# snt-arg/visual_sgraphs

Hardware: NVIDIA B200
Metric: orb_extraction_frames_per_s_640x480_1000f (higher is better)
Workload: dtype u8

## Files before the change

visual_sgraphs_b200/csrc/fast.cu:

```cuda
#include "blur_device.cuh"
#include "vsg_internal.cuh"

namespace vsg {

__device__ __forceinline__ uint32_t min2(uint32_t a, uint32_t b) { uint32_t d; asm("min.u16x2 %0, %1, %2;" : "=r"(d) : "r"(a), "r"(b)); return d; }
__device__ __forceinline__ uint32_t max2(uint32_t a, uint32_t b) { uint32_t d; asm("max.u16x2 %0, %1, %2;" : "=r"(d) : "r"(a), "r"(b)); return d; }
__device__ __forceinline__ uint32_t min3(uint32_t a, uint32_t b, uint32_t c) { return min2(min2(a, b), c); }
__device__ __forceinline__ uint32_t max3(uint32_t a, uint32_t b, uint32_t c) { return max2(max2(a, b), c); }

constexpr int kFastThreads = 160;
#ifndef VSG_FAST_MINB
#define VSG_FAST_MINB 6
#endif
constexpr int kT2Pitch = 52;
constexpr int kS2Pitch = 52;
constexpr int kMaxS = 28;

__device__ __forceinline__ uint32_t fast_strength2(const uint32_t *c) {
    constexpr int P = kT2Pitch;
    uint32_t p[16];
    p[0] = c[3 * P];       p[1] = c[3 * P + 1];    p[2] = c[2 * P + 2];    p[3] = c[P + 3];
    p[4] = c[3];           p[5] = c[-P + 3];       p[6] = c[-2 * P + 2];   p[7] = c[-3 * P + 1];
    p[8] = c[-3 * P];      p[9] = c[-3 * P - 1];   p[10] = c[-2 * P - 2];  p[11] = c[-P - 3];
    p[12] = c[-3];         p[13] = c[P - 3];       p[14] = c[2 * P - 2];   p[15] = c[3 * P - 1];
    const uint32_t v = c[0];
    uint32_t glo[4], ghi[4];
#pragma unroll
    for (int g = 0; g < 4; ++g) {
        const int b = 4 * g;
        const uint32_t s0 = p[b], s1 = p[b + 1], s2 = p[b + 2], s3 = p[(b + 9) & 15], s4 = p[(b + 10) & 15], s5 = p[(b + 11) & 15];
        const uint32_t q0 = p[b + 3], q1 = p[(b + 4) & 15], q2 = p[(b + 5) & 15], q3 = p[(b + 6) & 15], q4 = p[(b + 7) & 15], q5 = p[(b + 8) & 15];
        glo[g] = min3(max2(min3(max2(s0, s3), s1, s2), min3(max2(s2, s5), s3, s4)), min3(q0, q1, q2), min3(q3, q4, q5));
        ghi[g] = max3(min2(max3(min2(s0, s3), s1, s2), max3(min2(s2, s5), s3, s4)), max3(q0, q1, q2), max3(q3, q4, q5));
    }
    const uint32_t best_lo = max3(glo[0], glo[1], max2(glo[2], glo[3]));
    const uint32_t best_hi = min3(ghi[0], ghi[1], min2(ghi[2], ghi[3]));
    return max2(max2(best_lo, v) - v, v - min2(best_hi, v));
}

__constant__ uint32_t kRcpS[kMaxS / 4 + 1] = {0u, 0x40000000u, 0x20000000u, 0x15555556u, 0x10000000u, 0x0CCCCCCDu, 0x0AAAAAABu, 0x0924924Au};
__constant__ uint8_t kRowsPerSweep[kMaxS / 4 + 1] = {0, 40, 20, 13, 10, 8, 6, 5};

struct CellGeom {
    int level, x0, y0, cw, ch;
};
__device__ __forceinline__ CellGeom cell_geom(const FrameGeom &g, int cell_block) {
    CellGeom c;
    int level = 0;
#pragma unroll
    for (int l = 1; l < 8; ++l) level += cell_block >= g.lv[l].cell_begin ? 1 : 0;
    for (int l = 8; l < g.nlevels; ++l) level += cell_block >= g.lv[l].cell_begin ? 1 : 0;
    const LevelGeom &L = g.lv[level];
    const int local = cell_block - L.cell_begin;
    const int ci = (int)__umulhi((uint32_t)local, L.cols_rcp), cj = local - ci * L.cols_eff;
    c.level = level;
    c.x0 = kBorderMin + cj * L.w_cell;
    c.y0 = kBorderMin + ci * L.h_cell;
    c.cw = min(c.x0 + L.w_cell + 6, L.w - kBorderMin) - c.x0;
    c.ch = min(c.y0 + L.h_cell + 6, L.h - kBorderMin) - c.y0;
    return c;
}

__device__ __forceinline__ void fast_cell_body(const FrameGeom &g, const CellGeom &cell, const uint8_t *__restrict__ lvl0_base,
                                               int lvl0_pitch, int64_t lvl0_stride, const uint8_t *__restrict__ pyr,
                                               uint32_t *t2, uint32_t *s2, uint32_t *list, Cand *__restrict__ cand,
                                               int *__restrict__ cand_count, int ini_th, int min_th, int list_cap, int frame) {
    __shared__ int s_count, s_base;
    const int level = cell.level, x0 = cell.x0, y0 = cell.y0, cw = cell.cw, ch = cell.ch;
    const LevelGeom &L = g.lv[level];
    const int tid = threadIdx.x;
    const int iw = cw - 6, ih = ch - 6;
    const int S = (((iw + 1) >> 1) + 3) & ~3;
    const int ax0 = x0 & ~3;
    const int xoff = x0 - ax0;
    {
        const int nq = (xoff + S + 6 + 3) >> 2;
        const int lq = nq <= 8 ? 3 : 4;
        const int q = tid & ((1 << lq) - 1), r0 = tid >> lq, rstep = kFastThreads >> lq;
        const bool qok = q < nq;
        auto relayout = [&](uint32_t a, uint32_t b, uint32_t *dst) {
            uint4 o;
            o.x = __byte_perm(a, b, 0x7470) & 0x00FF00FFu;
            o.y = __byte_perm(a, b, 0x7571) & 0x00FF00FFu;
            o.z = __byte_perm(a, b, 0x7672) & 0x00FF00FFu;
            o.w = __byte_perm(a, b, 0x7773) & 0x00FF00FFu;
            *reinterpret_cast<uint4 *>(dst) = o;
        };
        const uint8_t *src;
        int spitch;
        if (level == 0) { src = lvl0_base + (int64_t)frame * lvl0_stride; spitch = lvl0_pitch; }
        else { src = pyr + L.plane_offset + (int64_t)frame * L.plane_stride; spitch = L.pitch; }
        const uint8_t *base = src + (int64_t)y0 * spitch + ax0;
        const uint8_t *row = base + (int64_t)r0 * spitch + 4 * q;
        const int64_t rinc = (int64_t)rstep * spitch;
        uint32_t *dst = t2 + r0 * kT2Pitch + 4 * q;
        constexpr int kLoadIters = 3;
        uint32_t a[kLoadIters], b[kLoadIters];
#pragma unroll
        for (int it = 0; it < kLoadIters; ++it) {
            if (qok && r0 + it * rstep < ch) {
                a[it] = __ldg(reinterpret_cast<const uint32_t *>(row + it * rinc));
                b[it] = __ldg(reinterpret_cast<const uint32_t *>(row + it * rinc + S));
            }
        }
#pragma unroll
        for (int it = 0; it < kLoadIters; ++it)
            if (qok && r0 + it * rstep < ch) relayout(a[it], b[it], dst + it * rstep * kT2Pitch);
        for (int r = r0 + kLoadIters * rstep; qok && r < ch; r += rstep) {
            const uint8_t *rp = base + (int64_t)r * spitch + 4 * q;
            relayout(__ldg(reinterpret_cast<const uint32_t *>(rp)), __ldg(reinterpret_cast<const uint32_t *>(rp + S)),
                     t2 + r * kT2Pitch + 4 * q);
        }
    }
    for (int i = tid; i < kS2Pitch; i += kFastThreads) {
        s2[i] = 0;
        s2[(ih + 1) * kS2Pitch + i] = 0;
    }
    if (tid == 0) s_count = 0;

    const int RB = kRowsPerSweep[S >> 2];
    const int trow = (int)__umulhi((uint32_t)tid, kRcpS[S >> 2]);
    const int j = tid - trow * S;
    const int row0 = trow < RB ? trow : ih;
    const uint32_t kmask = (j < iw ? 0x0000FFFFu : 0u) | (j + S < iw ? 0xFFFF0000u : 0u);
    __syncthreads();

    {
        const uint32_t *c = t2 + (3 + row0) * kT2Pitch + xoff + 3 + j;
        uint32_t *k = s2 + (row0 + 1) * kS2Pitch + j + 1;
        const bool first = j == 0, last = j == S - 1;
        for (int row = row0; row < ih; row += RB, c += RB * kT2Pitch, k += RB * kS2Pitch) {
            const uint32_t K = fast_strength2(c) & kmask;
            *k = K;
            if (last) k[-S] = K << 16;
            if (first) k[S] = K >> 16;
        }
    }
    __syncthreads();

    for (int pass = 0; pass < 2; ++pass) {
        const int t = pass == 0 ? ini_th : min_th;
        const int tt = max(t, 1);
        const uint32_t tt2 = (uint32_t)tt * 0x00010001u;
        uint32_t acc = 0, pw = 1;
        const uint32_t *c = s2 + (row0 + 1) * kS2Pitch + j + 1;
        for (int row = row0; row < ih; row += RB, c += RB * kS2Pitch, pw <<= 1) {
            const uint32_t K = c[0];
            const uint32_t nb = max3(max3(c[-kS2Pitch - 1], c[-kS2Pitch], c[-kS2Pitch + 1]),
                                     max3(c[-1], c[1], c[kS2Pitch - 1]), max3(c[kS2Pitch], c[kS2Pitch + 1], tt2));
            const uint32_t e = K - min2(K, nb);
            acc += min2(e, 0x00010001u) * pw;
        }
        const int cnt = __popc(acc);
        if (cnt) {
            int pos = atomicAdd(&s_count, cnt);
            uint32_t m0 = acc & 0xFFFFu, m1 = acc >> 16;
            const uint32_t *kcol = s2 + (row0 + 1) * kS2Pitch + j + 1;
            while (m0) {
                const int i = __ffs(m0) - 1;
                m0 &= m0 - 1;
                const uint32_t K = kcol[i * RB * kS2Pitch] & 0xFFFFu;
                list[pos++] = (uint32_t)j | ((uint32_t)(row0 + i * RB) << 8) | ((K - 1) << 16);
            }
            while (m1) {
                const int i = __ffs(m1) - 1;
                m1 &= m1 - 1;
                const uint32_t K = kcol[i * RB * kS2Pitch] >> 16;
                list[pos++] = (uint32_t)(j + S) | ((uint32_t)(row0 + i * RB) << 8) | ((K - 1) << 16);
            }
        }
        __syncthreads();
        if (s_count > 0) break;
    }
    const int n = min(s_count, list_cap);
    if (n == 0) return;
    const int slot_idx = frame * g.nlevels + level;
    if (tid == 0) s_base = atomicAdd(&cand_count[slot_idx], n);
    __syncthreads();
    Cand *out = cand + L.cand_offset + (int64_t)frame * g.cand_total;
    for (int i = tid; i < n; i += kFastThreads) {
        const int dst = s_base + i;
        if (dst >= L.cand_cap) break;
        const uint32_t e = list[i];
        Cand c;
        c.x = (unsigned short)(x0 + 3 + (e & 0xff));
        c.y = (unsigned short)(y0 + 3 + ((e >> 8) & 0xff));
        c.score = (unsigned short)(e >> 16);
        c.pad = 0;
        out[dst] = c;
    }
}

struct FastSmem {
    uint32_t *t2, *s2, *list;
};
__device__ __forceinline__ FastSmem fast_smem(uint8_t *base, int tile_rows) {
    FastSmem m;
    m.t2 = reinterpret_cast<uint32_t *>(base);
    m.s2 = m.t2 + tile_rows * kT2Pitch;
    m.list = m.s2 + (tile_rows - 4) * kS2Pitch;
    return m;
}

__global__ void __launch_bounds__(kFastThreads, VSG_FAST_MINB) fast_kernel(FrameGeom g,
                                                             const uint8_t *__restrict__ lvl0_base, int lvl0_pitch,
                                                             int64_t lvl0_stride, const uint8_t *__restrict__ pyr,
                                                             Cand *__restrict__ cand, int *__restrict__ cand_count,
                                                             int ini_th, int min_th, int tile_rows, int list_cap) {
    extern __shared__ __align__(16) uint8_t smem[];
    pdl_launch_dependents();
    pdl_wait();
    const FastSmem m = fast_smem(smem, tile_rows);
    fast_cell_body(g, cell_geom(g, blockIdx.x), lvl0_base, lvl0_pitch, lvl0_stride, pyr, m.t2, m.s2, m.list, cand,
                   cand_count, ini_th, min_th, list_cap, blockIdx.y);
}

struct UnitRole {
    bool blur;
    int index;
};
__device__ __forceinline__ UnitRole unit_role(int x, int nblur, int ratio, uint32_t group_rcp) {
    const int group = ratio + 1;
    UnitRole r;
    if (x < nblur * group) {
        const int gi = group == 1 ? x : (int)__umulhi((uint32_t)x, group_rcp), pos = x - gi * group;
        r.blur = pos == ratio;
        r.index = r.blur ? gi : gi * ratio + pos;
    } else {
        r.blur = false;
        r.index = nblur * ratio + (x - nblur * group);
    }
    return r;
}

__global__ void __launch_bounds__(kFastThreads, VSG_FAST_MINB) fast_blur_kernel(FrameGeom g, BlurLevels bl,
                                                                  const uint8_t *__restrict__ lvl0_base, int lvl0_pitch,
                                                                  int64_t lvl0_stride, const uint8_t *__restrict__ pyr,
                                                                  uint8_t *__restrict__ blur, Cand *__restrict__ cand,
                                                                  int *__restrict__ cand_count, int ini_th, int min_th,
                                                                  int tile_rows, int list_cap, int nblur, int ratio,
                                                                  uint32_t group_rcp) {
    extern __shared__ __align__(16) uint8_t smem[];
    pdl_launch_dependents();
    pdl_wait();
    const UnitRole role = unit_role(blockIdx.x, nblur, ratio, group_rcp);
    if (role.blur) {
        blur_block_body(g, bl, lvl0_base, lvl0_pitch, lvl0_stride, pyr, blur, role.index, blockIdx.y);
        return;
    }
    const FastSmem m = fast_smem(smem, tile_rows);
    fast_cell_body(g, cell_geom(g, role.index), lvl0_base, lvl0_pitch, lvl0_stride, pyr, m.t2, m.s2, m.list, cand,
                   cand_count, ini_th, min_th, list_cap, blockIdx.y);
}

vsg_status launch_fast(const FrameGeom &g, const uint8_t *lvl0_base, int lvl0_pitch, int64_t lvl0_stride, const uint8_t *pyr,
                       uint8_t *blur, Cand *cand, int *cand_count, int ini_th, int min_th, int max_cw, int max_ch, int nframes,
                       cudaStream_t s) {
    if (g.ncells == 0) {
        if (blur) launch_blur(g, lvl0_base, lvl0_pitch, lvl0_stride, pyr, blur, nframes, s);
        return VSG_OK;
    }
    const int max_S = ((((max_cw - 6) + 1) >> 1) + 3) & ~3;
    if (3 + max_S + 6 + 3 > kT2Pitch || max_S + 2 > kS2Pitch || max_S > kMaxS || (max_ch - 6) > 16 * (kFastThreads / max_S)) {
        set_error("FAST cell larger than the shared-memory tile / the 16-sweep survivor masks");
        return VSG_ERR_INVALID;
    }
    const int tile_rows = max_ch;
    const int list_cap = ((max_cw - 6 + 1) / 2) * ((max_ch - 6 + 1) / 2) + 1;
    const size_t smem = (size_t)tile_rows * kT2Pitch * 4 + (size_t)(tile_rows - 4) * kS2Pitch * 4 + (size_t)list_cap * 4 + 16;
    if (smem > 48 * 1024) {
        cudaFuncSetAttribute(fast_kernel, cudaFuncAttributeMaxDynamicSharedMemorySize, (int)smem);
        cudaFuncSetAttribute(fast_blur_kernel, cudaFuncAttributeMaxDynamicSharedMemorySize, (int)smem);
    }
    if (!blur) {
        launch_kernel(fast_kernel, dim3(g.ncells, nframes), dim3(kFastThreads), smem, s, true, g, lvl0_base, lvl0_pitch,
                      lvl0_stride, pyr, cand, cand_count, ini_th, min_th, tile_rows, list_cap);
    } else {
        const BlurLevels bl = make_blur_levels(g, nframes, kFastThreads);
        const int nblur = bl.block_begin[g.nlevels];
        const int ratio = g.ncells / nblur;
        const uint32_t group_rcp = (uint32_t)((0x100000000ull + (uint64_t)ratio) / (uint64_t)(ratio + 1));
        launch_kernel(fast_blur_kernel, dim3(g.ncells + nblur, nframes), dim3(kFastThreads), smem, s, true, g, bl, lvl0_base,
                      lvl0_pitch, lvl0_stride, pyr, blur, cand, cand_count, ini_th, min_th, tile_rows, list_cap, nblur, ratio,
                      group_rcp);
    }
    count_launch();
    return VSG_OK;
}

}
```

visual_sgraphs_b200/csrc/vsg_api.cu:

```cuda
#include <algorithm>
#include <atomic>
#include <cmath>
#include <cstdarg>
#include <cstdio>
#include <cstdlib>
#include <cstring>
#include <vector>

#include "vsg_internal.cuh"

namespace vsg {

static thread_local char g_err[512] = "";
static std::atomic<int64_t> g_launches{0};

void set_error(const char *fmt, ...) {
    va_list ap;
    va_start(ap, fmt);
    vsnprintf(g_err, sizeof(g_err), fmt, ap);
    va_end(ap);
}
bool cuda_ok(cudaError_t e, const char *what) {
    if (e == cudaSuccess) return true;
    set_error("%s: %s", what, cudaGetErrorString(e));
    return false;
}
void count_launch(int n) { g_launches += n; }
static thread_local bool g_pdl_small_batch = true;
constexpr int kPdlMaxFrames = 8;
void pdl_scope(int nframes) { g_pdl_small_batch = nframes <= kPdlMaxFrames; }
bool pdl_enabled() { return g_pdl_small_batch; }

static inline int cv_round(float v) { return (int)lrintf(v); }
static inline int cv_round(double v) { return (int)lrint(v); }
static inline int64_t align_up(int64_t v, int64_t a) { return (v + a - 1) / a * a; }

}

using namespace vsg;

struct vsg_extractor {
    int device = 0;
    int max_batch = 1;
    cudaStream_t stream = nullptr;
    static constexpr int kAuxStreams = 2;
    cudaStream_t aux[kAuxStreams] = {nullptr, nullptr};
    int chunk_frames = 128;
    uint8_t *color_d = nullptr;
    size_t color_bytes = 0;
    uint32_t *rect_xy[2] = {nullptr, nullptr};
    uint16_t *rect_frac[2] = {nullptr, nullptr};
    int rect_w = 0, rect_h = 0;
    cudaEvent_t fork_ev = nullptr;
    vsg_orb_params p{};
    std::vector<float> scale, inv_scale, sigma2, inv_sigma2;
    std::vector<int> quota;

    int cur_w = 0, cur_h = 0;
    FrameGeom g{};
    int max_cw = 0, max_ch = 0, max_nodes = 0;
    int64_t pyr_bytes_per_frame = 0;

    short4 *tabs_d = nullptr;
    PyrTile *pyr_tiles_d = nullptr;
    int pyr_ntiles = 0, pyr_tile_buf = 0;
    size_t pyr_tile_smem = 0;
    uint8_t *pyr = nullptr, *blur = nullptr;
    Cand *cand = nullptr;
    unsigned short *node_of = nullptr;
    int *cand_count = nullptr;
    LevelKp *level_kps = nullptr;
    int *level_kp_count = nullptr;
    int *slot = nullptr;
    uint8_t *out_block_d = nullptr, *out_block_h = nullptr;
    size_t out_block_bytes = 0;
    vsg_keypoint *kps_d = nullptr;
    uint8_t *desc_d = nullptr;
    int *n_d = nullptr, *mono_d = nullptr;
    vsg_keypoint *kps_h = nullptr;
    uint8_t *desc_h = nullptr;
    int *n_h = nullptr, *mono_h = nullptr;

    bool profile = false;
    static constexpr int kEvRing = 32;
    cudaEvent_t ev[kEvRing][VSG_NUM_STAGES + 1] = {};
    bool ev_created = false;
    int ev_head = 0, ev_pending = 0;
    double stage_ms[VSG_NUM_STAGES] = {0, 0, 0, 0, 0};
    int64_t stage_runs = 0;

    void harvest_one() {
        const int slot = (ev_head - ev_pending + 2 * kEvRing) % kEvRing;
        cudaEventSynchronize(ev[slot][VSG_NUM_STAGES]);
        for (int k = 0; k < VSG_NUM_STAGES; ++k) {
            float ms = 0.f;
            cudaEventElapsedTime(&ms, ev[slot][k], ev[slot][k + 1]);
            stage_ms[k] += ms;
        }
        ++stage_runs;
        --ev_pending;
    }

    const uint8_t *lvl0_base = nullptr;
    int lvl0_pitch = 0;
    int64_t lvl0_stride = 0;
    int last_nframes = 0;
    bool results_on_handle = false;

    void free_shape() {
        cudaFree(tabs_d); cudaFree(pyr_tiles_d); cudaFree(pyr); cudaFree(blur); cudaFree(cand); cudaFree(node_of);
        cudaFree(cand_count); cudaFree(level_kps); cudaFree(level_kp_count); cudaFree(slot); cudaFree(out_block_d);
        cudaFree(color_d);
        color_d = nullptr; color_bytes = 0;
        cudaFreeHost(out_block_h);
        out_block_d = out_block_h = nullptr; out_block_bytes = 0;
        tabs_d = nullptr; pyr_tiles_d = nullptr; pyr_ntiles = 0; pyr = blur = nullptr; cand = nullptr; node_of = nullptr;
        cand_count = nullptr; level_kps = nullptr; level_kp_count = nullptr; slot = nullptr; kps_d = nullptr;
        desc_d = nullptr; n_d = mono_d = nullptr; kps_h = nullptr; desc_h = nullptr; n_h = mono_h = nullptr;
        cur_w = cur_h = 0;
    }
};

namespace {

void build_tables(vsg_extractor *ex) {
    const int nl = ex->p.nlevels;
    const double scale_factor = ex->p.scale_factor;
    ex->scale.assign(nl, 1.f);
    ex->sigma2.assign(nl, 1.f);
    for (int i = 1; i < nl; ++i) {
        ex->scale[i] = (float)(ex->scale[i - 1] * scale_factor);
        ex->sigma2[i] = ex->scale[i] * ex->scale[i];
    }
    ex->inv_scale.resize(nl);
    ex->inv_sigma2.resize(nl);
    for (int i = 0; i < nl; ++i) {
        ex->inv_scale[i] = 1.0f / ex->scale[i];
        ex->inv_sigma2[i] = 1.0f / ex->sigma2[i];
    }
    ex->quota.assign(nl, 0);
    const float factor = (float)(1.0f / scale_factor);
    float desired = ex->p.nfeatures * (1 - factor) / (1 - (float)std::pow((double)factor, (double)nl));
    int sum = 0;
    for (int l = 0; l < nl - 1; ++l) {
        ex->quota[l] = cv_round(desired);
        sum += ex->quota[l];
        desired *= factor;
    }
    ex->quota[nl - 1] = std::max(ex->p.nfeatures - sum, 0);
}

void build_resize_tables(int sw, int sh, int dw, int dh, int dw_pad, std::vector<short4> &xt, std::vector<short4> &yt) {
    const double scale_x = 1.0 / ((double)dw / sw), scale_y = 1.0 / ((double)dh / sh);
    xt.resize(dw_pad);
    yt.resize(dh);
    for (int dx = 0; dx < dw_pad; ++dx) {
        const int x = std::min(dx, dw - 1);
        float fx = (float)((x + 0.5) * scale_x - 0.5);
        int sx = (int)std::floor(fx);
        fx -= sx;
        if (sx < 0) { fx = 0; sx = 0; }
        if (sx >= sw - 1) { fx = 0; sx = sw - 1; }
        xt[dx] = make_short4((short)sx, (short)std::min(sx + 1, sw - 1), (short)cv_round((1.f - fx) * 2048.f),
                             (short)cv_round(fx * 2048.f));
    }
    for (int dy = 0; dy < dh; ++dy) {
        float fy = (float)((dy + 0.5) * scale_y - 0.5);
        int sy = (int)std::floor(fy);
        fy -= sy;
        const int sy0 = std::min(std::max(sy, 0), sh - 1), sy1 = std::min(std::max(sy + 1, 0), sh - 1);
        yt[dy] = make_short4((short)sy0, (short)sy1, (short)cv_round((1.f - fy) * 2048.f), (short)cv_round(fy * 2048.f));
    }
}

vsg_status configure_shape(vsg_extractor *ex, int w, int h) {
    if (ex->cur_w == w && ex->cur_h == h) return VSG_OK;
    if (w > kMaxImageDim || h > kMaxImageDim) {
        set_error("image %dx%d too large: at most %d pixels per side", w, h, kMaxImageDim);
        return VSG_ERR_INVALID;
    }
    CK(cudaSetDevice(ex->device));
    int smem_optin = 0;
    size_t octree_static = 0;
    CK(cudaDeviceGetAttribute(&smem_optin, cudaDevAttrMaxSharedMemoryPerBlockOptin, ex->device));
    const vsg_status ost = octree_static_smem_bytes(&octree_static);
    if (ost != VSG_OK) return ost;
    ex->free_shape();
    const int nl = ex->p.nlevels;
    FrameGeom &g = ex->g;
    memset(&g, 0, sizeof(g));
    g.nlevels = nl;
    std::vector<Cell> cells;
    ex->max_cw = ex->max_ch = 7;
    ex->max_nodes = 8;
    int64_t plane_off = 0, cand_off = 0;
    int kp_off = 0;
    std::vector<std::vector<short4>> xts(nl), yts(nl);
    for (int l = 0; l < nl; ++l) {
        LevelGeom &L = g.lv[l];
        L.w = cv_round((float)w * ex->inv_scale[l]);
        L.h = cv_round((float)h * ex->inv_scale[l]);
        const int min_b = kBorderMin, max_bx = L.w - kBorderMin, max_by = L.h - kBorderMin;
        const float width = (float)(max_bx - min_b), height = (float)(max_by - min_b);
        if (width < 35.f || height < 35.f) {
            set_error("image %dx%d too small: level %d is %dx%d (needs >= 67x67 for one 35-px cell)", w, h, l, L.w, L.h);
            return VSG_ERR_INVALID;
        }
        L.pitch = (int)align_up(L.w, 64);
        L.plane_stride = align_up((int64_t)L.pitch * L.h, 256);
        L.plane_offset = plane_off;
        plane_off += L.plane_stride * ex->max_batch;
        L.n_cols = (int)(width / 35.f);
        L.n_rows = (int)(height / 35.f);
        L.w_cell = (int)std::ceil(width / L.n_cols);
        L.h_cell = (int)std::ceil(height / L.n_rows);
        L.cell_begin = (int)cells.size();
        int cand_cap = 0;
        for (int i = 0; i < L.n_rows; ++i) {
            const float ini_y = (float)(min_b + i * L.h_cell);
            float max_y = ini_y + L.h_cell + 6;
            if (ini_y >= max_by - 3) continue;
            if (max_y > max_by) max_y = (float)max_by;
            for (int j = 0; j < L.n_cols; ++j) {
                const float ini_x = (float)(min_b + j * L.w_cell);
                float max_x = ini_x + L.w_cell + 6;
                if (ini_x >= max_bx - 6) continue;
                if (max_x > max_bx) max_x = (float)max_bx;
                Cell c;
                c.level = (short)l;
                c.x0 = (short)ini_x; c.y0 = (short)ini_y;
                c.cw = (short)((int)max_x - (int)ini_x); c.ch = (short)((int)max_y - (int)ini_y);
                c.pad = 0;
                if (c.cw < 7 || c.ch < 7) continue;
                cells.push_back(c);
                ex->max_cw = std::max<int>(ex->max_cw, c.cw);
                ex->max_ch = std::max<int>(ex->max_ch, c.ch);
                cand_cap += ((c.cw - 6 + 1) / 2) * ((c.ch - 6 + 1) / 2);
            }
        }
        L.cell_count = (int)cells.size() - L.cell_begin;
        L.cols_eff = L.rows_eff = 0;
        for (int k = L.cell_begin; k < (int)cells.size(); ++k) {
            const Cell &c = cells[k];
            L.cols_eff = std::max(L.cols_eff, (c.x0 - min_b) / L.w_cell + 1);
            L.rows_eff = std::max(L.rows_eff, (c.y0 - min_b) / L.h_cell + 1);
        }
        if (L.cols_eff * L.rows_eff != L.cell_count) {
            set_error("internal: level %d cell table is not a prefix rectangle", l);
            return VSG_ERR_INVALID;
        }
        L.cols_rcp = (uint32_t)((0x100000000ull + (uint64_t)L.cols_eff - 1) / (uint64_t)std::max(L.cols_eff, 1));
        L.wcell_rcp = L.w_cell > 1 ? (uint32_t)((0x100000000ull + (uint64_t)L.w_cell - 1) / (uint64_t)L.w_cell) : 0xFFFFFFFFu;
        L.hcell_rcp = L.h_cell > 1 ? (uint32_t)((0x100000000ull + (uint64_t)L.h_cell - 1) / (uint64_t)L.h_cell) : 0xFFFFFFFFu;
        L.quota = ex->quota[l];
        L.n_ini = (int)std::round(static_cast<float>(max_bx - min_b) / (max_by - min_b));
        if (L.n_ini < 1) {
            set_error("image %dx%d: aspect ratio below 0.5 is not supported by the reference oct-tree (nIni = 0)", w, h);
            return VSG_ERR_INVALID;
        }
        L.h_x = static_cast<float>(max_bx - min_b) / L.n_ini;
        L.cand_cap = cand_cap + 8;
        L.cand_offset = cand_off;
        cand_off += L.cand_cap;
        L.kp_cap = std::max(L.quota, 4 * L.n_ini) + 4;
        L.kp_offset = kp_off;
        kp_off += L.kp_cap;
        const size_t octree_need = octree_smem_bytes(L.kp_cap + 4) + octree_static;
        if (octree_need > (size_t)smem_optin) {
            set_error("level %d: oct-tree quota %d needs %zu bytes of shared memory per block, the device allows %d", l, L.quota,
                      octree_need, smem_optin);
            return VSG_ERR_INVALID;
        }
        ex->max_nodes = std::max(ex->max_nodes, L.kp_cap + 4);
        L.scale = ex->scale[l];
        L.kp_size = (float)(int)(kPatch * ex->scale[l]);
        L.resize_tma_ok = 0;
        if (l > 0) {
            build_resize_tables(g.lv[l - 1].w, g.lv[l - 1].h, L.w, L.h, (int)align_up(L.w, 4), xts[l], yts[l]);
            L.resize_tma_ok = resize_tma_fits(xts[l], yts[l], L.w, L.h) ? 1 : 0;
        }
    }
    g.ncells = (int)cells.size();
    for (int l = nl; l < kMaxLevels; ++l) g.lv[l].cell_begin = 0x7fffffff;
    g.cand_total = cand_off;
    g.kp_total = kp_off;
    g.out_cap = kp_off;
    ex->pyr_bytes_per_frame = plane_off / ex->max_batch;

    const int B = ex->max_batch;
    size_t ntab = 0;
    for (int l = 1; l < nl; ++l) ntab += xts[l].size() + yts[l].size();
    CK(cudaMalloc(&ex->tabs_d, std::max<size_t>(ntab, 1) * sizeof(short4)));
    size_t toff = 0;
    for (int l = 1; l < nl; ++l) {
        CK(cudaMemcpy(ex->tabs_d + toff, xts[l].data(), xts[l].size() * sizeof(short4), cudaMemcpyHostToDevice));
        g.lv[l].xtab = ex->tabs_d + toff;
        toff += xts[l].size();
        CK(cudaMemcpy(ex->tabs_d + toff, yts[l].data(), yts[l].size() * sizeof(short4), cudaMemcpyHostToDevice));
        g.lv[l].ytab = ex->tabs_d + toff;
        toff += yts[l].size();
    }
    if (nl >= 2) {
        constexpr int ntx = 12, nty = 12;
        std::vector<PyrTile> tiles((size_t)ntx * nty);
        int buf = 0, ntab_max = 0, dim_max = 0;
        for (int ty = 0; ty < nty; ++ty)
            for (int tx = 0; tx < ntx; ++tx) {
                PyrTile &t = tiles[(size_t)ty * ntx + tx];
                int ntab_t = 0;
                for (int l = nl - 1; l >= 0; --l) {
                    const int W = g.lv[l].w, H = g.lv[l].h;
                    PyrTileBox o{(short)(tx * W / ntx), (short)(ty * H / nty), (short)((tx + 1) * W / ntx - 1), (short)((ty + 1) * H / nty - 1)};
                    PyrTileBox r = o;
                    if (l < nl - 1) {
                        const PyrTileBox &u = t.region[l + 1];
                        const short nx0 = xts[l + 1][u.x0].x, nx1 = xts[l + 1][u.x1].y, ny0 = yts[l + 1][u.y0].x, ny1 = yts[l + 1][u.y1].y;
                        if (l == 0) r = PyrTileBox{nx0, ny0, nx1, ny1};
                        else r = PyrTileBox{std::min(o.x0, nx0), std::min(o.y0, ny0), std::max(o.x1, nx1), std::max(o.y1, ny1)};
                    }
                    t.owned[l] = o;
                    t.region[l] = r;
                    t.rcp_w[l] = (uint32_t)((0x100000000ull + (uint64_t)(r.x1 - r.x0)) / (uint64_t)(r.x1 - r.x0 + 1));
                    buf = std::max(buf, (r.x1 - r.x0 + 1) * (r.y1 - r.y0 + 1));
                    if (l > 0) dim_max = std::max(dim_max, std::max(r.x1 - r.x0 + 1, r.y1 - r.y0 + 1));
                    if (l > 0) ntab_t += (r.x1 - r.x0 + 1) + (r.y1 - r.y0 + 1);
                }
                for (int l = nl; l < kMaxLevels; ++l) { t.owned[l] = t.region[l] = PyrTileBox{0, 0, -1, -1}; t.rcp_w[l] = 0; }
                ntab_max = std::max(ntab_max, ntab_t);
            }
        ex->pyr_tile_buf = (int)align_up(buf, 16);
        ex->pyr_tile_smem = 2 * (size_t)ex->pyr_tile_buf + (size_t)ntab_max * sizeof(short4);
        if (ex->pyr_tile_smem <= 160 * 1024 && dim_max <= 256 && buf < 65536 && nl <= kMaxLevels && g.lv[nl - 1].w >= 2 * ntx && g.lv[nl - 1].h >= 2 * nty) {
            CK(cudaMalloc(&ex->pyr_tiles_d, tiles.size() * sizeof(PyrTile)));
            CK(cudaMemcpy(ex->pyr_tiles_d, tiles.data(), tiles.size() * sizeof(PyrTile), cudaMemcpyHostToDevice));
            ex->pyr_ntiles = (int)tiles.size();
        }
    }
    CK(cudaMalloc(&ex->pyr, plane_off + 256));
    CK(cudaMalloc(&ex->blur, plane_off + 256));
    CK(cudaMemset(ex->pyr, 0, plane_off + 256));
    CK(cudaMalloc(&ex->cand, (size_t)g.cand_total * B * sizeof(Cand)));
    CK(cudaMalloc(&ex->node_of, (size_t)g.cand_total * B * sizeof(unsigned short)));
    CK(cudaMalloc(&ex->cand_count, (size_t)B * nl * sizeof(int)));
    CK(cudaMalloc(&ex->level_kps, (size_t)g.kp_total * B * sizeof(LevelKp)));
    CK(cudaMalloc(&ex->level_kp_count, (size_t)B * nl * sizeof(int)));
    CK(cudaMalloc(&ex->slot, (size_t)g.kp_total * B * sizeof(int)));
    {
        auto up = [](size_t v) { return (v + 255) & ~(size_t)255; };
        const size_t off_desc = up((size_t)g.out_cap * B * sizeof(vsg_keypoint));
        const size_t off_n = off_desc + up((size_t)g.out_cap * B * 32);
        const size_t off_mono = off_n + up((size_t)B * sizeof(int));
        ex->out_block_bytes = off_mono + up((size_t)B * sizeof(int));
        CK(cudaMalloc(&ex->out_block_d, ex->out_block_bytes));
        CK(cudaMallocHost(&ex->out_block_h, ex->out_block_bytes));
        ex->kps_d = reinterpret_cast<vsg_keypoint *>(ex->out_block_d);
        ex->desc_d = ex->out_block_d + off_desc;
        ex->n_d = reinterpret_cast<int *>(ex->out_block_d + off_n);
        ex->mono_d = reinterpret_cast<int *>(ex->out_block_d + off_mono);
        ex->kps_h = reinterpret_cast<vsg_keypoint *>(ex->out_block_h);
        ex->desc_h = ex->out_block_h + off_desc;
        ex->n_h = reinterpret_cast<int *>(ex->out_block_h + off_n);
        ex->mono_h = reinterpret_cast<int *>(ex->out_block_h + off_mono);
    }
    ex->cur_w = w;
    ex->cur_h = h;
    return VSG_OK;
}

static int pyr_tile_max_frames() {
    const char *e = getenv("VSG_PYR_TILE");
    return e ? atoi(e) : 4;
}

vsg_status run_pipeline(vsg_extractor *ex, cudaStream_t s, int f0, const uint8_t *lvl0_base, int lvl0_pitch,
                        int64_t lvl0_stride, int nframes, int lap_x0, int lap_x1, vsg_keypoint *kps_dev,
                        uint8_t *desc_dev, int out_cap, int *n_dev, int *mono_dev) {
    FrameGeom g = ex->g;
    for (int l = 0; l < g.nlevels; ++l) {
        g.lv[l].plane_offset += (int64_t)f0 * g.lv[l].plane_stride;
        g.lv[l].cand_offset += (int64_t)f0 * g.cand_total;
    }
    pdl_scope(nframes);
    int *cand_count = ex->cand_count + (size_t)f0 * g.nlevels;
    int *level_kp_count = ex->level_kp_count + (size_t)f0 * g.nlevels;
    LevelKp *level_kps = ex->level_kps + (size_t)f0 * g.kp_total;
    int *slot = ex->slot + (size_t)f0 * g.kp_total;
    CK(cudaMemsetAsync(cand_count, 0, (size_t)nframes * g.nlevels * sizeof(int), s));
    cudaEvent_t *ev = nullptr;
    if (ex->profile && s == ex->stream) {
        if (!ex->ev_created) {
            for (int i = 0; i < vsg_extractor::kEvRing; ++i)
                for (int k = 0; k <= VSG_NUM_STAGES; ++k) CK(cudaEventCreate(&ex->ev[i][k]));
            ex->ev_created = true;
        }
        if (ex->ev_pending == vsg_extractor::kEvRing) ex->harvest_one();
        ev = ex->ev[ex->ev_head];
        ex->ev_head = (ex->ev_head + 1) % vsg_extractor::kEvRing;
        ++ex->ev_pending;
    }
#define STAGE_MARK(k) do { if (ev) CK(cudaEventRecord(ev[k], s)); } while (0)
    STAGE_MARK(0);
    if (ex->pyr_tiles_d && nframes <= pyr_tile_max_frames()) {
        launch_pyramid_tiles(g, ex->pyr_tiles_d, ex->pyr_ntiles, ex->pyr_tile_buf, ex->pyr_tile_smem, lvl0_base, lvl0_pitch, lvl0_stride,
                             ex->pyr, nframes, s);
    } else {
        for (int l = 1; l < g.nlevels; ++l) {
            const LevelGeom &P = g.lv[l - 1];
            if (l == 1) launch_resize_level(g, l, lvl0_base, lvl0_pitch, lvl0_stride, ex->pyr, nframes, s);
            else launch_resize_level(g, l, ex->pyr + P.plane_offset, P.pitch, P.plane_stride, ex->pyr, nframes, s);
        }
    }
    STAGE_MARK(1);
    const BlurTcPlan *blur_tc = plan_blur_tc(g, lvl0_base, lvl0_pitch, lvl0_stride, ex->pyr, ex->blur, nframes);
    const vsg_status fst = launch_fast(g, lvl0_base, lvl0_pitch, lvl0_stride, ex->pyr, blur_tc ? nullptr : ex->blur, ex->cand,
                                       cand_count, ex->p.ini_th_fast, ex->p.min_th_fast, ex->max_cw, ex->max_ch, nframes, s);
    if (fst != VSG_OK) return fst;
    STAGE_MARK(2);
    const vsg_status ost = launch_octree(g, ex->cand, cand_count, ex->node_of, level_kps, level_kp_count, ex->max_nodes, nframes, s);
    if (ost != VSG_OK) return ost;
    STAGE_MARK(3);
    if (blur_tc) launch_blur_tc(blur_tc, ex->blur, s);
    STAGE_MARK(4);
    launch_describe(g, lvl0_base, lvl0_pitch, lvl0_stride, ex->pyr, ex->blur, level_kps, level_kp_count, lap_x0,
                    lap_x1, kps_dev, desc_dev, out_cap, n_dev, mono_dev, slot, nframes, s);
    STAGE_MARK(5);
#undef STAGE_MARK
    CK(cudaGetLastError());
    return VSG_OK;
}

}

namespace vsg {
bool extractor_pyramid(vsg_extractor *ex, PyramidRef *out) {
    if (!ex || ex->cur_w == 0 || ex->last_nframes == 0) return false;
    out->device = ex->device;
    out->nframes = ex->last_nframes;
    out->geom = &ex->g;
    out->lvl0_base = ex->lvl0_base;
    out->lvl0_pitch = ex->lvl0_pitch;
    out->lvl0_stride = ex->lvl0_stride;
    out->pyr = ex->pyr;
    out->scale = ex->scale.data();
    out->inv_scale = ex->inv_scale.data();
    out->stream = ex->stream;
// ... 416 lines not shown
```

visual_sgraphs_b200/csrc/vsg_internal.cuh:

```cuda
#pragma once
#include <cuda_runtime.h>
#include <stdint.h>

#include <vector>

#include "../../include/vsg_cuda.h"

namespace vsg {

constexpr int kMaxLevels = 16;
constexpr int kEdge = 19;
constexpr int kBorderMin = 16;
constexpr int kMaxImageDim = 16384;
constexpr int kHalfPatch = 15;
constexpr int kPatch = 31;

struct LevelGeom {
    int w, h;
    int pitch;
    int64_t plane_stride;
    int64_t plane_offset;
    int n_cols, n_rows, w_cell, h_cell;
    int cell_begin, cell_count;
    int cols_eff, rows_eff;
    uint32_t cols_rcp;
    uint32_t wcell_rcp, hcell_rcp;
    int quota;
    int n_ini;
    float h_x;
    int cand_cap;
    int64_t cand_offset;
    int kp_cap;
    int kp_offset;
    float scale;
    float kp_size;
    int resize_tma_ok;
    const short4 *xtab;
    const short4 *ytab;
};

struct FrameGeom {
    int nlevels;
    int ncells;
    int64_t cand_total;
    int kp_total;
    int out_cap;
    LevelGeom lv[kMaxLevels];
};

struct Cell {
    short level;
    short x0, y0;
    short cw, ch;
    short pad;
};

struct __align__(8) Cand {
    unsigned short x, y;
    unsigned short score;
    unsigned short pad;
};

struct __align__(8) LevelKp {
    unsigned short x, y;
    unsigned short score;
    unsigned short pad;
};

}

struct vsg_matcher {
    int device = 0;
    cudaStream_t stream = nullptr;
    void *buf[20] = {};
    size_t cap[20] = {};
    void *hbuf[8] = {};
    size_t hcap[8] = {};
    std::vector<char> scratch[2];
    int sm_count = 148;
};

namespace vsg {

vsg_status matcher_ensure(vsg_matcher *m, int slot, size_t bytes);
vsg_status matcher_ensure_host(vsg_matcher *m, int slot, size_t bytes);
vsg_status launch_knn2_merge_parts(vsg_matcher *m, const int32_t *idx_parts, const int32_t *dist_parts, int nparts, int nq,
                                   int32_t *out_idx, int32_t *out_dist);
bool knn2_tc_supported(int nq, int nt);
vsg_status knn2_tc_device(vsg_matcher *m, const uint8_t *q_dev, int nq, const uint8_t *t_dev, int nt, int offset, int *idx_dev,
                          int *dist_dev);
void launch_window_dists(vsg_matcher *m, const uint8_t *query_dev, int nq, const uint8_t *train_dev,
                         const int *cand_ptr_dev, const int *cand_dev, int *all_dist_dev);

struct PyramidRef {
    int device;
    int nframes;
    const FrameGeom *geom;
    const uint8_t *lvl0_base;
    int lvl0_pitch;
    int64_t lvl0_stride;
    const uint8_t *pyr;
    const float *scale, *inv_scale;
    cudaStream_t stream;
    const vsg_keypoint *kps_dev;
    const uint8_t *desc_dev;
    const int *n_dev;
    int out_cap;
};
bool extractor_pyramid(vsg_extractor *ex, PyramidRef *out);

__device__ __forceinline__ void pdl_launch_dependents() { asm volatile("griddepcontrol.launch_dependents;" ::: "memory"); }
__device__ __forceinline__ void pdl_wait() { asm volatile("griddepcontrol.wait;" ::: "memory"); }
bool pdl_enabled();
void pdl_scope(int nframes);

template <class... KArgs, class... Args>
inline cudaError_t launch_kernel(void (*kernel)(KArgs...), dim3 grid, dim3 block, size_t smem, cudaStream_t s, bool pdl,
                                 Args... args) {
    cudaLaunchConfig_t cfg = {};
    cfg.gridDim = grid;
    cfg.blockDim = block;
    cfg.dynamicSmemBytes = smem;
    cfg.stream = s;
    cudaLaunchAttribute attr[1];
    attr[0].id = cudaLaunchAttributeProgrammaticStreamSerialization;
    attr[0].val.programmaticStreamSerializationAllowed = 1;
    cfg.attrs = attr;
    cfg.numAttrs = (pdl && pdl_enabled()) ? 1 : 0;
    return cudaLaunchKernelEx(&cfg, kernel, KArgs(args)...);
}

void set_error(const char *fmt, ...);
bool cuda_ok(cudaError_t e, const char *what);
#define CK(call)                                          \
    do {                                                  \
        if (!cuda_ok((call), #call)) return VSG_ERR_CUDA; \
    } while (0)
void count_launch(int n = 1);

struct PyrTileBox { short x0, y0, x1, y1; };
struct PyrTile {
    PyrTileBox region[kMaxLevels], owned[kMaxLevels];
    uint32_t rcp_w[kMaxLevels];
};
void launch_pyramid_tiles(const FrameGeom &g, const PyrTile *tiles, int ntiles, int buf_bytes, size_t smem, const uint8_t *lvl0_base,
                          int lvl0_pitch, int64_t lvl0_stride, uint8_t *pyr, int nframes, cudaStream_t s);
bool launch_resize_level_tma(const FrameGeom &g, int level, const uint8_t *src_base, int src_pitch, int64_t src_stride, uint8_t *pyr,
                             int nframes, cudaStream_t s);
bool resize_tma_fits(const std::vector<short4> &xt, const std::vector<short4> &yt, int dw, int dh);
void launch_resize_level(const FrameGeom &g, int level, const uint8_t *src_base, int src_pitch, int64_t src_stride,
                         uint8_t *pyr, int nframes, cudaStream_t s);
void launch_cvt_gray(const uint8_t *src, int src_pitch, int64_t src_stride, int channels, int r_first, uint8_t *dst,
                     int dst_pitch, int64_t dst_stride, int w, int h, int nframes, cudaStream_t s);
struct RectifyMaps {
    const uint32_t *xy[2];
    const uint16_t *frac[2];
    int nslots;
};
void launch_remap(const uint8_t *src, int src_pitch, int64_t src_stride, int sw, int sh, const RectifyMaps &maps, int first_frame,
                  uint8_t *dst, int dst_pitch, int64_t dst_stride, int w, int h, int nframes, cudaStream_t s);
struct BlurTcPlan;
const BlurTcPlan *plan_blur_tc(const FrameGeom &g, const uint8_t *lvl0_base, int lvl0_pitch, int64_t lvl0_stride, const uint8_t *pyr,
                               const uint8_t *blur, int nframes);
void launch_blur_tc(const BlurTcPlan *plan, uint8_t *blur, cudaStream_t s);
void launch_blur(const FrameGeom &g, const uint8_t *lvl0_base, int lvl0_pitch, int64_t lvl0_stride, const uint8_t *pyr,
                 uint8_t *blur, int nframes, cudaStream_t s);
vsg_status launch_fast(const FrameGeom &g, const uint8_t *lvl0_base, int lvl0_pitch, int64_t lvl0_stride, const uint8_t *pyr,
                       uint8_t *blur, Cand *cand, int *cand_count, int ini_th, int min_th, int max_cw, int max_ch, int nframes,
                       cudaStream_t s);
size_t octree_smem_bytes(int max_nodes);
vsg_status octree_static_smem_bytes(size_t *bytes);
vsg_status launch_octree(const FrameGeom &g, const Cand *cand, const int *cand_count, unsigned short *node_of,
                         LevelKp *level_kps, int *level_kp_count, int max_nodes, int nframes, cudaStream_t s);
void launch_describe(const FrameGeom &g, const uint8_t *lvl0_base, int lvl0_pitch, int64_t lvl0_stride,
                     const uint8_t *pyr, const uint8_t *blur, const LevelKp *level_kps, const int *level_kp_count,
                     int lap_x0, int lap_x1, vsg_keypoint *kps_out, uint8_t *desc_out, int out_cap, int *n_out,
                     int *mono_out, int *slot_scratch, int nframes, cudaStream_t s);

}
```

Measured before the change: 157,300.

## Precompute per-cell FAST geometry in a device table and bump occupancy bounds

Replaces the per-block level search and division that derived cell geometry with a 16-byte precomputed FastCell record loaded once per block. The record carries sweep row count, stride reciprocal and sweep count, so the FAST loops iterate a fixed count. The load path switches to 32-bit offsets with predicated stores. The FAST kernel's min-blocks launch bound rises from 6 to 7, which may force register spills. An optional frame-major grid ordering is added behind a macro.

```diff
diff --git a/visual_sgraphs_b200/csrc/fast.cu b/visual_sgraphs_b200/csrc/fast.cu
--- a/visual_sgraphs_b200/csrc/fast.cu
+++ b/visual_sgraphs_b200/csrc/fast.cu
@@ -9,9 +9,8 @@
 __device__ __forceinline__ uint32_t max3(uint32_t a, uint32_t b, uint32_t c) { return max2(max2(a, b), c); }
 
 constexpr int kFastThreads = 160;
-#ifndef VSG_FAST_MINB
-#define VSG_FAST_MINB 6
-#endif
+constexpr int kFastMinBlocks = 7;
+constexpr int kFastBlurMinBlocks = 6;
 constexpr int kT2Pitch = 52;
 constexpr int kS2Pitch = 52;
 constexpr int kMaxS = 28;
@@ -38,39 +37,32 @@
     return max2(max2(best_lo, v) - v, v - min2(best_hi, v));
 }
 
-__constant__ uint32_t kRcpS[kMaxS / 4 + 1] = {0u, 0x40000000u, 0x20000000u, 0x15555556u, 0x10000000u, 0x0CCCCCCDu, 0x0AAAAAABu, 0x0924924Au};
-__constant__ uint8_t kRowsPerSweep[kMaxS / 4 + 1] = {0, 40, 20, 13, 10, 8, 6, 5};
-
-struct CellGeom {
-    int level, x0, y0, cw, ch;
-};
-__device__ __forceinline__ CellGeom cell_geom(const FrameGeom &g, int cell_block) {
-    CellGeom c;
-    int level = 0;
-#pragma unroll
-    for (int l = 1; l < 8; ++l) level += cell_block >= g.lv[l].cell_begin ? 1 : 0;
-    for (int l = 8; l < g.nlevels; ++l) level += cell_block >= g.lv[l].cell_begin ? 1 : 0;
-    const LevelGeom &L = g.lv[level];
-    const int local = cell_block - L.cell_begin;
-    const int ci = (int)__umulhi((uint32_t)local, L.cols_rcp), cj = local - ci * L.cols_eff;
-    c.level = level;
-    c.x0 = kBorderMin + cj * L.w_cell;
-    c.y0 = kBorderMin + ci * L.h_cell;
-    c.cw = min(c.x0 + L.w_cell + 6, L.w - kBorderMin) - c.x0;
-    c.ch = min(c.y0 + L.h_cell + 6, L.h - kBorderMin) - c.y0;
+FastCell make_fast_cell(int level, int x0, int y0, int cw, int ch) {
+    FastCell c;
+    const int S = (((cw - 6 + 1) >> 1) + 3) & ~3, rb = kFastThreads / S;
+    c.x0 = (unsigned short)x0;
+    c.y0 = (unsigned short)y0;
+    c.cw = (unsigned short)cw;
+    c.ch = (unsigned short)ch;
+    c.level = (unsigned char)level;
+    c.S = (unsigned char)S;
+    c.rb = (unsigned char)rb;
+    c.nsw = (unsigned char)((ch - 6 + rb - 1) / rb);
+    c.rcp_s = (uint32_t)((0x100000000ull + (uint64_t)S - 1) / (uint64_t)S);
     return c;
 }
 
-__device__ __forceinline__ void fast_cell_body(const FrameGeom &g, const CellGeom &cell, const uint8_t *__restrict__ lvl0_base,
+__device__ __forceinline__ void fast_cell_body(const FrameGeom &g, int cell_index, const uint8_t *__restrict__ lvl0_base,
                                                int lvl0_pitch, int64_t lvl0_stride, const uint8_t *__restrict__ pyr,
                                                uint32_t *t2, uint32_t *s2, uint32_t *list, Cand *__restrict__ cand,
                                                int *__restrict__ cand_count, int ini_th, int min_th, int list_cap, int frame) {
     __shared__ int s_count, s_base;
-    const int level = cell.level, x0 = cell.x0, y0 = cell.y0, cw = cell.cw, ch = cell.ch;
+    FastCell cell;
+    *reinterpret_cast<uint4 *>(&cell) = __ldg(reinterpret_cast<const uint4 *>(g.cells) + cell_index);
+    const int level = cell.level, x0 = cell.x0, y0 = cell.y0, cw = cell.cw, ch = cell.ch, S = cell.S;
     const LevelGeom &L = g.lv[level];
     const int tid = threadIdx.x;
     const int iw = cw - 6, ih = ch - 6;
-    const int S = (((iw + 1) >> 1) + 3) & ~3;
     const int ax0 = x0 & ~3;
     const int xoff = x0 - ax0;
     {
@@ -78,39 +70,43 @@
         const int lq = nq <= 8 ? 3 : 4;
         const int q = tid & ((1 << lq) - 1), r0 = tid >> lq, rstep = kFastThreads >> lq;
         const bool qok = q < nq;
-        auto relayout = [&](uint32_t a, uint32_t b, uint32_t *dst) {
+        auto relayout = [](uint32_t a, uint32_t b) {
             uint4 o;
             o.x = __byte_perm(a, b, 0x7470) & 0x00FF00FFu;
             o.y = __byte_perm(a, b, 0x7571) & 0x00FF00FFu;
             o.z = __byte_perm(a, b, 0x7672) & 0x00FF00FFu;
             o.w = __byte_perm(a, b, 0x7773) & 0x00FF00FFu;
-            *reinterpret_cast<uint4 *>(dst) = o;
+            return o;
         };
         const uint8_t *src;
         int spitch;
         if (level == 0) { src = lvl0_base + (int64_t)frame * lvl0_stride; spitch = lvl0_pitch; }
         else { src = pyr + L.plane_offset + (int64_t)frame * L.plane_stride; spitch = L.pitch; }
-        const uint8_t *base = src + (int64_t)y0 * spitch + ax0;
-        const uint8_t *row = base + (int64_t)r0 * spitch + 4 * q;
-        const int64_t rinc = (int64_t)rstep * spitch;
+        const uint8_t *pa = src + (int64_t)y0 * spitch + ax0 + 4 * q;
+        const uint8_t *pb = pa + S;
+        const uint32_t rinc = (uint32_t)(rstep * spitch);
+        uint32_t off = (uint32_t)(r0 * spitch);
         uint32_t *dst = t2 + r0 * kT2Pitch + 4 * q;
         constexpr int kLoadIters = 3;
-        uint32_t a[kLoadIters], b[kLoadIters];
+        uint32_t a[kLoadIters] = {}, b[kLoadIters] = {};
+        bool ok[kLoadIters];
 #pragma unroll
         for (int it = 0; it < kLoadIters; ++it) {
-            if (qok && r0 + it * rstep < ch) {
-                a[it] = __ldg(reinterpret_cast<const uint32_t *>(row + it * rinc));
-                b[it] = __ldg(reinterpret_cast<const uint32_t *>(row + it * rinc + S));
+            ok[it] = qok && r0 + it * rstep < ch;
+            if (ok[it]) {
+                a[it] = __ldg(reinterpret_cast<const uint32_t *>(pa + off + it * rinc));
+                b[it] = __ldg(reinterpret_cast<const uint32_t *>(pb + off + it * rinc));
             }
         }
 #pragma unroll
-        for (int it = 0; it < kLoadIters; ++it)
-            if (qok && r0 + it * rstep < ch) relayout(a[it], b[it], dst + it * rstep * kT2Pitch);
-        for (int r = r0 + kLoadIters * rstep; qok && r < ch; r += rstep) {
-            const uint8_t *rp = base + (int64_t)r * spitch + 4 * q;
-            relayout(__ldg(reinterpret_cast<const uint32_t *>(rp)), __ldg(reinterpret_cast<const uint32_t *>(rp + S)),
-                     t2 + r * kT2Pitch + 4 * q);
-        }
+        for (int it = 0; it < kLoadIters; ++it) {
+            const uint4 o = relayout(a[it], b[it]);
+            if (ok[it]) *reinterpret_cast<uint4 *>(dst + it * rstep * kT2Pitch) = o;
+        }
+        off += kLoadIters * rinc;
+        for (int r = r0 + kLoadIters * rstep; qok && r < ch; r += rstep, off += rinc)
+            *reinterpret_cast<uint4 *>(t2 + r * kT2Pitch + 4 * q) =
+                relayout(__ldg(reinterpret_cast<const uint32_t *>(pa + off)), __ldg(reinterpret_cast<const uint32_t *>(pb + off)));
     }
     for (int i = tid; i < kS2Pitch; i += kFastThreads) {
         s2[i] = 0;
@@ -118,10 +114,11 @@
     }
     if (tid == 0) s_count = 0;
 
-    const int RB = kRowsPerSweep[S >> 2];
-    const int trow = (int)__umulhi((uint32_t)tid, kRcpS[S >> 2]);
+    const int RB = cell.rb;
+    const int trow = (int)__umulhi((uint32_t)tid, cell.rcp_s);
     const int j = tid - trow * S;
-    const int row0 = trow < RB ? trow : ih;
+    const int row0 = trow < RB ? trow : 0;
+    const int nsw = trow < RB ? cell.nsw - (trow >= ih - (cell.nsw - 1) * RB ? 1 : 0) : 0;
     const uint32_t kmask = (j < iw ? 0x0000FFFFu : 0u) | (j + S < iw ? 0xFFFF0000u : 0u);
     __syncthreads();
 
@@ -129,7 +126,7 @@
         const uint32_t *c = t2 + (3 + row0) * kT2Pitch + xoff + 3 + j;
         uint32_t *k = s2 + (row0 + 1) * kS2Pitch + j + 1;
         const bool first = j == 0, last = j == S - 1;
-        for (int row = row0; row < ih; row += RB, c += RB * kT2Pitch, k += RB * kS2Pitch) {
+        for (int sw = 0; sw < nsw; ++sw, c += RB * kT2Pitch, k += RB * kS2Pitch) {
             const uint32_t K = fast_strength2(c) & kmask;
             *k = K;
             if (last) k[-S] = K << 16;
@@ -144,7 +141,7 @@
         const uint32_t tt2 = (uint32_t)tt * 0x00010001u;
         uint32_t acc = 0, pw = 1;
         const uint32_t *c = s2 + (row0 + 1) * kS2Pitch + j + 1;
-        for (int row = row0; row < ih; row += RB, c += RB * kS2Pitch, pw <<= 1) {
+        for (int sw = 0; sw < nsw; ++sw, c += RB * kS2Pitch, pw <<= 1) {
             const uint32_t K = c[0];
             const uint32_t nb = max3(max3(c[-kS2Pitch - 1], c[-kS2Pitch], c[-kS2Pitch + 1]),
                                      max3(c[-1], c[1], c[kS2Pitch - 1]), max3(c[kS2Pitch], c[kS2Pitch + 1], tt2));
@@ -202,7 +199,7 @@
     return m;
 }
 
-__global__ void __launch_bounds__(kFastThreads, VSG_FAST_MINB) fast_kernel(FrameGeom g,
+__global__ void __launch_bounds__(kFastThreads, kFastMinBlocks) fast_kernel(FrameGeom g,
                                                              const uint8_t *__restrict__ lvl0_base, int lvl0_pitch,
                                                              int64_t lvl0_stride, const uint8_t *__restrict__ pyr,
                                                              Cand *__restrict__ cand, int *__restrict__ cand_count,
@@ -211,8 +208,13 @@
     pdl_launch_dependents();
     pdl_wait();
     const FastSmem m = fast_smem(smem, tile_rows);
-    fast_cell_body(g, cell_geom(g, blockIdx.x), lvl0_base, lvl0_pitch, lvl0_stride, pyr, m.t2, m.s2, m.list, cand,
+#ifdef VSG_FAST_FRAME_MAJOR
+    fast_cell_body(g, blockIdx.y, lvl0_base, lvl0_pitch, lvl0_stride, pyr, m.t2, m.s2, m.list, cand,
+                   cand_count, ini_th, min_th, list_cap, blockIdx.x);
+#else
+    fast_cell_body(g, blockIdx.x, lvl0_base, lvl0_pitch, lvl0_stride, pyr, m.t2, m.s2, m.list, cand,
                    cand_count, ini_th, min_th, list_cap, blockIdx.y);
+#endif
 }
 
 struct UnitRole {
@@ -233,7 +235,7 @@
     return r;
 }
 
-__global__ void __launch_bounds__(kFastThreads, VSG_FAST_MINB) fast_blur_kernel(FrameGeom g, BlurLevels bl,
+__global__ void __launch_bounds__(kFastThreads, kFastBlurMinBlocks) fast_blur_kernel(FrameGeom g, BlurLevels bl,
                                                                   const uint8_t *__restrict__ lvl0_base, int lvl0_pitch,
                                                                   int64_t lvl0_stride, const uint8_t *__restrict__ pyr,
                                                                   uint8_t *__restrict__ blur, Cand *__restrict__ cand,
@@ -249,7 +251,7 @@
         return;
     }
     const FastSmem m = fast_smem(smem, tile_rows);
-    fast_cell_body(g, cell_geom(g, role.index), lvl0_base, lvl0_pitch, lvl0_stride, pyr, m.t2, m.s2, m.list, cand,
+    fast_cell_body(g, role.index, lvl0_base, lvl0_pitch, lvl0_stride, pyr, m.t2, m.s2, m.list, cand,
                    cand_count, ini_th, min_th, list_cap, blockIdx.y);
 }
 
@@ -273,7 +275,12 @@
         cudaFuncSetAttribute(fast_blur_kernel, cudaFuncAttributeMaxDynamicSharedMemorySize, (int)smem);
     }
     if (!blur) {
-        launch_kernel(fast_kernel, dim3(g.ncells, nframes), dim3(kFastThreads), smem, s, true, g, lvl0_base, lvl0_pitch,
+#ifdef VSG_FAST_FRAME_MAJOR
+        launch_kernel(fast_kernel, dim3(nframes, g.ncells),
+#else
+        launch_kernel(fast_kernel, dim3(g.ncells, nframes),
+#endif
+                       dim3(kFastThreads), smem, s, true, g, lvl0_base, lvl0_pitch,
                       lvl0_stride, pyr, cand, cand_count, ini_th, min_th, tile_rows, list_cap);
     } else {
         const BlurLevels bl = make_blur_levels(g, nframes, kFastThreads);
diff --git a/visual_sgraphs_b200/csrc/vsg_api.cu b/visual_sgraphs_b200/csrc/vsg_api.cu
--- a/visual_sgraphs_b200/csrc/vsg_api.cu
+++ b/visual_sgraphs_b200/csrc/vsg_api.cu
@@ -62,6 +62,7 @@
     int64_t pyr_bytes_per_frame = 0;
 
     short4 *tabs_d = nullptr;
+    FastCell *cells_d = nullptr;
     PyrTile *pyr_tiles_d = nullptr;
     int pyr_ntiles = 0, pyr_tile_buf = 0;
     size_t pyr_tile_smem = 0;
@@ -108,13 +109,13 @@
     bool results_on_handle = false;
 
     void free_shape() {
-        cudaFree(tabs_d); cudaFree(pyr_tiles_d); cudaFree(pyr); cudaFree(blur); cudaFree(cand); cudaFree(node_of);
+        cudaFree(tabs_d); cudaFree(cells_d); cudaFree(pyr_tiles_d); cudaFree(pyr); cudaFree(blur); cudaFree(cand); cudaFree(node_of);
         cudaFree(cand_count); cudaFree(level_kps); cudaFree(level_kp_count); cudaFree(slot); cudaFree(out_block_d);
         cudaFree(color_d);
         color_d = nullptr; color_bytes = 0;
         cudaFreeHost(out_block_h);
         out_block_d = out_block_h = nullptr; out_block_bytes = 0;
-        tabs_d = nullptr; pyr_tiles_d = nullptr; pyr_ntiles = 0; pyr = blur = nullptr; cand = nullptr; node_of = nullptr;
+        tabs_d = nullptr; cells_d = nullptr; pyr_tiles_d = nullptr; pyr_ntiles = 0; pyr = blur = nullptr; cand = nullptr; node_of = nullptr;
         cand_count = nullptr; level_kps = nullptr; level_kp_count = nullptr; slot = nullptr; kps_d = nullptr;
         desc_d = nullptr; n_d = mono_d = nullptr; kps_h = nullptr; desc_h = nullptr; n_h = mono_h = nullptr;
         cur_w = cur_h = 0;
@@ -190,7 +191,7 @@
     FrameGeom &g = ex->g;
     memset(&g, 0, sizeof(g));
     g.nlevels = nl;
-    std::vector<Cell> cells;
+    std::vector<FastCell> cells;
     ex->max_cw = ex->max_ch = 7;
     ex->max_nodes = 8;
     int64_t plane_off = 0, cand_off = 0;
@@ -214,7 +215,6 @@
         L.n_rows = (int)(height / 35.f);
         L.w_cell = (int)std::ceil(width / L.n_cols);
         L.h_cell = (int)std::ceil(height / L.n_rows);
-        L.cell_begin = (int)cells.size();
         int cand_cap = 0;
         for (int i = 0; i < L.n_rows; ++i) {
             const float ini_y = (float)(min_b + i * L.h_cell);
@@ -226,30 +226,14 @@
                 float max_x = ini_x + L.w_cell + 6;
                 if (ini_x >= max_bx - 6) continue;
                 if (max_x > max_bx) max_x = (float)max_bx;
-                Cell c;
-                c.level = (short)l;
-                c.x0 = (short)ini_x; c.y0 = (short)ini_y;
-                c.cw = (short)((int)max_x - (int)ini_x); c.ch = (short)((int)max_y - (int)ini_y);
-                c.pad = 0;
-                if (c.cw < 7 || c.ch < 7) continue;
-                cells.push_back(c);
-                ex->max_cw = std::max<int>(ex->max_cw, c.cw);
-                ex->max_ch = std::max<int>(ex->max_ch, c.ch);
-                cand_cap += ((c.cw - 6 + 1) / 2) * ((c.ch - 6 + 1) / 2);
+                const int cw = (int)max_x - (int)ini_x, ch = (int)max_y - (int)ini_y;
+                if (cw < 7 || ch < 7) continue;
+                cells.push_back(make_fast_cell(l, (int)ini_x, (int)ini_y, cw, ch));
+                ex->max_cw = std::max(ex->max_cw, cw);
+                ex->max_ch = std::max(ex->max_ch, ch);
+                cand_cap += ((cw - 6 + 1) / 2) * ((ch - 6 + 1) / 2);
             }
         }
-        L.cell_count = (int)cells.size() - L.cell_begin;
-        L.cols_eff = L.rows_eff = 0;
-        for (int k = L.cell_begin; k < (int)cells.size(); ++k) {
-            const Cell &c = cells[k];
-            L.cols_eff = std::max(L.cols_eff, (c.x0 - min_b) / L.w_cell + 1);
-            L.rows_eff = std::max(L.rows_eff, (c.y0 - min_b) / L.h_cell + 1);
-        }
-        if (L.cols_eff * L.rows_eff != L.cell_count) {
-            set_error("internal: level %d cell table is not a prefix rectangle", l);
-            return VSG_ERR_INVALID;
-        }
-        L.cols_rcp = (uint32_t)((0x100000000ull + (uint64_t)L.cols_eff - 1) / (uint64_t)std::max(L.cols_eff, 1));
         L.wcell_rcp = L.w_cell > 1 ? (uint32_t)((0x100000000ull + (uint64_t)L.w_cell - 1) / (uint64_t)L.w_cell) : 0xFFFFFFFFu;
         L.hcell_rcp = L.h_cell > 1 ? (uint32_t)((0x100000000ull + (uint64_t)L.h_cell - 1) / (uint64_t)L.h_cell) : 0xFFFFFFFFu;
         L.quota = ex->quota[l];
@@ -281,7 +265,6 @@
         }
     }
     g.ncells = (int)cells.size();
-    for (int l = nl; l < kMaxLevels; ++l) g.lv[l].cell_begin = 0x7fffffff;
     g.cand_total = cand_off;
     g.kp_total = kp_off;
     g.out_cap = kp_off;
@@ -291,6 +274,9 @@
     size_t ntab = 0;
     for (int l = 1; l < nl; ++l) ntab += xts[l].size() + yts[l].size();
     CK(cudaMalloc(&ex->tabs_d, std::max<size_t>(ntab, 1) * sizeof(short4)));
+    CK(cudaMalloc(&ex->cells_d, std::max<size_t>(cells.size(), 1) * sizeof(FastCell)));
+    CK(cudaMemcpy(ex->cells_d, cells.data(), cells.size() * sizeof(FastCell), cudaMemcpyHostToDevice));
+    g.cells = ex->cells_d;
     size_t toff = 0;
     for (int l = 1; l < nl; ++l) {
         CK(cudaMemcpy(ex->tabs_d + toff, xts[l].data(), xts[l].size() * sizeof(short4), cudaMemcpyHostToDevice));
diff --git a/visual_sgraphs_b200/csrc/vsg_internal.cuh b/visual_sgraphs_b200/csrc/vsg_internal.cuh
--- a/visual_sgraphs_b200/csrc/vsg_internal.cuh
+++ b/visual_sgraphs_b200/csrc/vsg_internal.cuh
@@ -21,9 +21,6 @@
     int64_t plane_stride;
     int64_t plane_offset;
     int n_cols, n_rows, w_cell, h_cell;
-    int cell_begin, cell_count;
-    int cols_eff, rows_eff;
-    uint32_t cols_rcp;
     uint32_t wcell_rcp, hcell_rcp;
     int quota;
     int n_ini;
@@ -39,20 +36,25 @@
     const short4 *ytab;
 };
 
+struct __align__(16) FastCell {
+    unsigned short x0, y0;
+    unsigned short cw, ch;
+    unsigned char level;
+    unsigned char S;
+    unsigned char rb;
+    unsigned char nsw;
+    uint32_t rcp_s;
+};
+FastCell make_fast_cell(int level, int x0, int y0, int cw, int ch);
+
 struct FrameGeom {
     int nlevels;
     int ncells;
     int64_t cand_total;
     int kp_total;
     int out_cap;
+    const FastCell *cells;
     LevelGeom lv[kMaxLevels];
-};
-
-struct Cell {
-    short level;
-    short x0, y0;
-    short cw, ch;
-    short pad;
 };
 
 struct __align__(8) Cand {
```

After: 160,700 (median of 6 runs). 2.2% higher.
